# stelleg/caster-dta

Hardware: AMD Instinct MI355X
Metric: graph-pairs/sec (Davis-shaped protein+drug), encoders fwd+bwd (higher is better)
Workload: dtype f32; 1 GPU; davis_b64; pairs_per_gpu=64, residues_per_gpu=19200, protein_edges_per_gpu=57484, atoms_per_gpu=2560, drug_edges_per_gpu=7986, encoder=CASTER-DTA(2,2), pass=fwdbwd, activation_storage=fp32, scope=encoders, torch_compile=False, tunable_gemms=False, two_lane_head=False, train_mode=True, csr_build_in_step=True, hip_graph=True, kernels=mfma

## Files before the change

### caster-dta_amd/csrc/gine_quad_kernels.hip

```cpp
#include <hip/hip_runtime.h>
#include <stdlib.h>
#include <stdint.h>

#include "gvp_internal.h"
#include "gvp_quad.h"

using namespace gq;

namespace {

constexpr int WAVE = 64, TILE = 16;
constexpr int NTL = 4;

constexpr int pad4i(int x) { return (x + 3) / 4 * 4; }

__device__ __forceinline__ int opaque_lane(int lane) {
  asm volatile("" : "+v"(lane));
  return lane;
}

#ifndef CGVP_GINE_FENCE
#define CGVP_GINE_FENCE 1
#endif
#if CGVP_GINE_FENCE
// ... 15 lines not shown
__device__ unsigned long long* g_stamp_buf_gine = nullptr;
#define GSTAMP(slot)                                                                         \
  do {                                                                                       \
    __builtin_amdgcn_sched_barrier(0);                                                       \
    unsigned long long t_;                                                                   \
    asm volatile("s_waitcnt vmcnt(0) lgkmcnt(0)\n\ts_memtime %0\n\ts_waitcnt lgkmcnt(0)" : "=s"(t_)::"memory"); \
    __builtin_amdgcn_sched_barrier(0);                                                       \
    if (g_stamp_buf_gine && (threadIdx.x & 63) == 0)                                         \
      g_stamp_buf_gine[((size_t)blockIdx.x * (blockDim.x >> 6) + (threadIdx.x >> 6)) * 16 + (slot)] = t_;   \
  } while (0)
#else
#define GSTAMP(slot) do {} while (0)
#endif

template <int W, int VALID>
struct SegClip {
  static_assert(W % 16 == 0, "whole 16-channel tiles");
  static constexpr int steps = W / 4;
  static __host__ __device__ int col(int s, int g) {
    const int c = 16 * (s >> 2) + 4 * g + (s & 3);
    return c < VALID ? c : -1;
  }
};

struct GineQArgs {
  const float* x; const int64_t* ntypes; const float* eattr; const int64_t* etypes;
  const int32_t* rowptr; const int32_t* eperm; const int32_t* esrc; const int32_t* edst; int64_t N;
  const float* eps; const float* we; const float* be; const float* w0; const float* b0;
  const float* w1; const float* b1; float slope;
  const float* mask; gvp::RngArgs rng; const float* g_out; float* g_x; float* slab;
  const float* agg_in; const uint16_t* pos_in;
  float* g_edge; float* g_self;
  float* g_eattr; int eattr_accum;
};

template <int COUT>
__device__ __forceinline__ f4 gine_dropout(const float* mask, const gvp::RngArgs& rng, int64_t n, int mt, int g) {
  if (mask) return *reinterpret_cast<const f4*>(mask + n * COUT + 16 * mt + 4 * g);
  if (rng.seed) {
    float f[4];
    gvp::dropout4(rng.seed[0], rng.seed[1], rng.stream, n, 4 * mt + g, rng.p, f);
    return f4{f[0], f[1], f[2], f[3]};
  }
  return f4{1.f, 1.f, 1.f, 1.f};
}

template <int CIN, int CHID, int COUT, int NT, int NET, int ED, bool EG = false>
struct GineQ {
  static_assert(CHID % 16 == 0 && COUT % 16 == 0 && COUT <= 64, "hidden / output widths are whole 16-channel tiles (<= 4 output tiles)");
  static constexpr int KE = NET + ED, XW = CIN - NT, CINP = (CIN + 15) / 16 * 16;
  static constexpr int MI = CINP / 16, MH = CHID / 16, MO = COUT / 16;
  static constexpr int L_EPS = 0, L_W0 = 1, L_B0 = L_W0 + CHID * CIN, L_W1 = L_B0 + CHID, L_B1 = L_W1 + COUT * CHID,
                       L_WE = L_B1 + COUT, L_BE = L_WE + CIN * KE, L_SIZE = L_BE + CIN, BLK = pad4i(L_SIZE);
  typedef SegClip<CINP, CIN> KIn;
  typedef Seg<P1, 0, CHID> KHid;
  typedef Seg<P1, 0, COUT> KOut;
  typedef Seg<P2, 0, KE> KFeat;
  static_assert(KFeat::steps <= 4, "bond one-hot + features fit one slot tile");
  typedef Gemm<P1, CIN, KE, KFeat> GE;
  typedef Gemm<P1, CHID, CIN, KIn> G0;
  typedef Gemm<P1, COUT, CHID, KHid> G1;
  typedef GemmT<KHid, KOut, CHID> G1T;
  typedef GemmT<KIn, KHid, CIN> G0T;
  typedef GemmT<KFeat, KIn, KE> GET;
  static_assert(GET::MT == 1, "d eattr is one output tile");
  static constexpr int F_E = 0, F_0 = F_E + GE::NFRAG * 64, F_0T = F_0 + G0::NFRAG * 64, F_1 = F_0T + G0T::NFRAG * 64,
// ... 282 lines not shown
#pragma unroll
      for (int mt = 0; mt < MI; ++mt) {
        f4 ag;
        if (SAVED) {
          ag = *reinterpret_cast<const f4*>(a.agg_in + (valid ? n : n0) * CINP + 16 * mt + 4 * g);
          if (!valid) ag = zero;
        } else {
          ag = *reinterpret_cast<const f4*>(rows + i * CINP + 16 * mt + 4 * g);
        }
#pragma unroll
        for (int r = 0; r < 4; ++r) h[mt][r] = fmaf(eps1, xi[mt][r], ag[r]);
      }
      float bh[1][Q::KIn::steps];
#pragma unroll
      for (int s = 0; s < Q::KIn::steps; ++s) bh[0][s] = h[s >> 2][s & 3];
      f4 tpre[MH], t[MH];
#pragma unroll
      for (int mt = 0; mt < MH; ++mt) {
        f4 acc[1] = {*reinterpret_cast<const f4*>(frag + Q::V_B0 + 16 * mt + 4 * g)};
        apply<typename Q::G0, 1>(frag + Q::F_0, mt, bh, acc, lane);
        tpre[mt] = acc[0];
#pragma unroll
        for (int r = 0; r < 4; ++r) t[mt][r] = acc[0][r] > 0.f ? acc[0][r] : acc[0][r] * a.slope;
      }
      float bt[1][Q::KHid::steps];
#pragma unroll
      for (int s = 0; s < Q::KHid::steps; ++s) bt[0][s] = t[s >> 2][s & 3];
      f4 dy[MO];
#pragma unroll
      for (int mt = 0; mt < MO; ++mt) {
        f4 acc[1] = {*reinterpret_cast<const f4*>(frag + Q::V_B1 + 16 * mt + 4 * g)};
        apply<typename Q::G1, 1>(frag + Q::F_1, mt, bt, acc, lane);
        f4 gy = *reinterpret_cast<const f4*>(a.g_out + (valid ? n : n0) * COUT + 16 * mt + 4 * g);
        gy = gy * gine_dropout<COUT>(a.mask, a.rng, valid ? n : n0, mt, g);
        if (!valid) gy = zero;
#pragma unroll
        for (int r = 0; r < 4; ++r) dy[mt][r] = gy[r] * (acc[0][r] > 0.f ? 1.f : a.slope);
      }
      float bdy[1][Q::KOut::steps];
#pragma unroll
      for (int s = 0; s < Q::KOut::steps; ++s) bdy[0][s] = dy[s >> 2][s & 3];
      f4 dtp[MH];
#pragma unroll
      for (int mt = 0; mt < MH; ++mt) {
        f4 acc[1] = {zero};
        apply<typename Q::G1T, 1>(frag + Q::F_1T, mt, bdy, acc, lane);
#pragma unroll
        for (int r = 0; r < 4; ++r) dtp[mt][r] = acc[0][r] * (tpre[mt][r] > 0.f ? 1.f : a.slope);
      }
      float bdt[1][Q::KHid::steps];
#pragma unroll
      for (int s = 0; s < Q::KHid::steps; ++s) bdt[0][s] = dtp[s >> 2][s & 3];
      f4 dh[MI];
#pragma unroll
      for (int mt = 0; mt < MI; ++mt) {
        f4 acc[1] = {zero};
        apply<typename Q::G0T, 1>(frag + Q::F_0T, mt, bdt, acc, lane);
        dh[mt] = acc[0];
      }
      GSTAMP(3);
      {
        f4 AT[MO], BT[MH];
        transpose_slots<Q::KOut::steps>(bdy[0], AT, lane, tscr);
        transpose_slots<Q::KHid::steps>(bt[0], BT, lane, tscr);
        dw1_band<Q, 0>(AT, BT, blk, lane);
        dw1_band<Q, 1>(AT, BT, blk, lane);
// ... 141 lines not shown
#pragma unroll
          for (int r = 0; r < 4; ++r) {
            const int c = 16 * mt + 4 * g + r;
            tot[r] = row_total(dm[mt][r]);
            q[r] = blk + Q::L_BE + c;
            on[r] = i == 15 && c < CIN;
          }
          add_where<AccPriv, 4>(q, on, tot);
        }
      }
    }
    WAVE_LDS_SYNC();
  }
  GSTAMP(6);
  for (int off = 32; off > 0; off >>= 1) acc_eps += __shfl_down(acc_eps, off);
  if (lane0 == 0) blk[Q::L_EPS] += acc_eps;
  __syncthreads();
  float* out = a.slab + (size_t)blockIdx.x * Q::L_SIZE;
  for (int k = threadIdx.x; k < Q::L_SIZE; k += GQ_TPB) {
    float s = 0.f;
#pragma unroll
    for (int ww = 0; ww < GQ_WPB; ++ww) s += blocks[ww * Q::BLK + k];
    out[k] = s;
  }
  GSTAMP(7);
}

struct GineFArgs {
  const float* x; const int64_t* ntypes; const float* eattr; const int64_t* etypes;
  const int32_t* rowptr; const int32_t* eperm; const int32_t* esrc; const int32_t* edst; int64_t N;
  const float* eps; const float* we; const float* be; const float* w0; const float* b0;
  const float* w1; const float* b1; float slope; const float* mask; gvp::RngArgs rng; float* out;
  float* agg_out; uint16_t* pos_out;
};
#ifndef CGVP_GINE_FWD_WAVES
#define CGVP_GINE_FWD_WAVES 8
#endif
constexpr int GF_WPB = CGVP_GINE_FWD_WAVES, GF_TPB = WAVE * GF_WPB;

template <int CIN, int CHID, int COUT, int NT, int NET, int ED>
__global__ __launch_bounds__(GF_TPB) void gine_quad_fwd_kernel(GineFArgs a) {
  typedef GineQ<CIN, CHID, COUT, NT, NET, ED> Q;
  constexpr int KE = Q::KE, XW = Q::XW, CINP = Q::CINP, MI = Q::MI, MH = Q::MH, MO = Q::MO;
  constexpr int FE = 0, F0 = FE + Q::GE::NFRAG * 64, F1 = F0 + Q::G0::NFRAG * 64, VBE = F1 + Q::G1::NFRAG * 64,
                VB0 = VBE + CINP, VB1 = VB0 + CHID, FSZ = VB1 + COUT;
  extern __shared__ __attribute__((aligned(16))) float lds[];
  float* frag = lds;
  const int lane0 = threadIdx.x & 63, w = threadIdx.x >> 6;
  float* rows = frag + FSZ + w * Q::ROWS;
  stage_fragments<typename Q::GE, GF_TPB>(frag + FE, a.we);
  stage_fragments<typename Q::G0, GF_TPB>(frag + F0, a.w0);
  stage_fragments<typename Q::G1, GF_TPB>(frag + F1, a.w1);
  stage_biases<CIN, CINP, CHID, COUT, GF_TPB>(frag + VBE, frag + VB0, frag + VB1, a.be, a.b0, a.b1);
  __syncthreads();

  const f4 zero = {0.f, 0.f, 0.f, 0.f};
  const float eps1 = 1.0f + a.eps[0];
  const int64_t ntiles = (a.N + TILE - 1) / TILE;
  for (int64_t tile = (int64_t)blockIdx.x * GF_WPB + w; tile < ntiles; tile += (int64_t)gridDim.x * GF_WPB) {
    const int64_t n0 = tile * TILE;
    const int nn = (int)((a.N - n0 < TILE) ? (a.N - n0) : TILE);
    const int32_t e0 = a.rowptr[n0], e1 = a.rowptr[n0 + nn];
    for (int k = lane0; k < Q::ROWS / 4; k += WAVE) reinterpret_cast<f4*>(rows)[k] = zero;
    WAVE_LDS_SYNC();
    for (int32_t c0 = e0; c0 < e1; c0 += NTL * TILE) {
      const int lane = opaque_lane(lane0), i = lane & 15, g = lane >> 4;
// ... 44 lines not shown
    }
    {
      const int lane = opaque_lane(lane0), i = lane & 15, g = lane >> 4;
      const bool valid = i < nn;
      const int64_t n = n0 + i;
      float bh[1][Q::KIn::steps];
      f4 xi[MI];
      node_inputs<Q, CIN, NT, G_PIN>(a, n, valid, n0, g, xi);
#pragma unroll
      for (int mt = 0; mt < MI; ++mt) {
        const f4 ag = *reinterpret_cast<const f4*>(rows + i * CINP + 16 * mt + 4 * g);
        if (a.agg_out && valid) *reinterpret_cast<f4*>(a.agg_out + n * CINP + 16 * mt + 4 * g) = ag;
#pragma unroll
        for (int r = 0; r < 4; ++r) bh[0][4 * mt + r] = fmaf(eps1, xi[mt][r], ag[r]);
      }
      float bt[1][Q::KHid::steps];
#pragma unroll
      for (int mt = 0; mt < MH; ++mt) {
        f4 acc[1] = {*reinterpret_cast<const f4*>(frag + VB0 + 16 * mt + 4 * g)};
        apply<typename Q::G0, 1>(frag + F0, mt, bh, acc, lane);
#pragma unroll
        for (int r = 0; r < 4; ++r) bt[0][4 * mt + r] = acc[0][r] > 0.f ? acc[0][r] : acc[0][r] * a.slope;
      }
#pragma unroll
      for (int mt = 0; mt < MO; ++mt) {
        f4 acc[1] = {*reinterpret_cast<const f4*>(frag + VB1 + 16 * mt + 4 * g)};
        apply<typename Q::G1, 1>(frag + F1, mt, bt, acc, lane);
        f4 y;
#pragma unroll
        for (int r = 0; r < 4; ++r) y[r] = acc[0][r] > 0.f ? acc[0][r] : acc[0][r] * a.slope;
        if (valid) {
          y = y * gine_dropout<COUT>(a.mask, a.rng, n, mt, g);
          *reinterpret_cast<f4*>(a.out + n * COUT + 16 * mt + 4 * g) = y;
        }
      }
    }
    WAVE_LDS_SYNC();
  }
}

template <int CIN, int CHID, int COUT, int NT, int NET, int ED>
int launch_fwd(GineFArgs& a, hipStream_t st) {
  typedef GineQ<CIN, CHID, COUT, NT, NET, ED> Q;
  const int64_t tiles = (a.N + TILE - 1) / TILE;
  int64_t wgs = (tiles + GF_WPB - 1) / GF_WPB;
  static const int cap = [] {
    const char* e = getenv("CGVP_GINE_FWD_WGS");
    const int v = e ? atoi(e) : 0;
    return v >= 1 ? v : 1024;
  }();
  const int G = (int)(wgs < 1 ? 1 : (wgs > cap ? cap : wgs));
  const size_t lds = (size_t)((Q::GE::NFRAG + Q::G0::NFRAG + Q::G1::NFRAG) * 64 + Q::CINP + CHID + COUT + GF_WPB * Q::ROWS) * sizeof(float);
  CGVP_SET_DYN_LDS_ONCE((gine_quad_fwd_kernel<CIN, CHID, COUT, NT, NET, ED>), lds);
  hipLaunchKernelGGL((gine_quad_fwd_kernel<CIN, CHID, COUT, NT, NET, ED>), dim3(G), dim3(GF_TPB), lds, st, a);
  return 0;
}

template <int CIN, int CHID, int COUT, int NT, int NET, int ED>
int launch(GineQArgs& a, int cap, int* rows, int* row_len, hipStream_t st) {
  typedef GineQ<CIN, CHID, COUT, NT, NET, ED> Q;
  constexpr int GQ_WPB = Q::WPB, GQ_TPB = Q::TPB;
  const int64_t tiles = (a.N + TILE - 1) / TILE;
  int64_t wgs = (tiles + GQ_WPB - 1) / GQ_WPB;
  const int G = (int)(wgs < 1 ? 1 : (wgs > cap ? cap : wgs));
  if (a.g_eattr) {
    typedef GineQ<CIN, CHID, COUT, NT, NET, ED, true> QE;
    static_assert(QE::TPB == Q::TPB && QE::L_SIZE == Q::L_SIZE, "same workgroup shape and slab row");
    const size_t ldse = (size_t)QE::LDS_FLOATS * sizeof(float);
    if (a.g_edge) {
      if (!(a.agg_in && a.pos_in)) return CGVP_ERR_NONDETERMINISTIC;
      CGVP_SET_DYN_LDS_ONCE((gine_quad_bwd_kernel<CIN, CHID, COUT, NT, NET, ED, true, true, true>), ldse);
      hipLaunchKernelGGL((gine_quad_bwd_kernel<CIN, CHID, COUT, NT, NET, ED, true, true, true>), dim3(G), dim3(GQ_TPB), ldse, st, a);
    } else if (a.agg_in && a.pos_in) {
      CGVP_SET_DYN_LDS_ONCE((gine_quad_bwd_kernel<CIN, CHID, COUT, NT, NET, ED, true, false, true>), ldse);
      hipLaunchKernelGGL((gine_quad_bwd_kernel<CIN, CHID, COUT, NT, NET, ED, true, false, true>), dim3(G), dim3(GQ_TPB), ldse, st, a);
    } else {
      CGVP_SET_DYN_LDS_ONCE((gine_quad_bwd_kernel<CIN, CHID, COUT, NT, NET, ED, false, false, true>), ldse);
      hipLaunchKernelGGL((gine_quad_bwd_kernel<CIN, CHID, COUT, NT, NET, ED, false, false, true>), dim3(G), dim3(GQ_TPB), ldse, st, a);
    }
    *rows = G;
    *row_len = Q::L_SIZE;
    return 0;
  }
  const size_t lds = (size_t)Q::LDS_FLOATS * sizeof(float);
  if (a.g_edge) {
    if (!(a.agg_in && a.pos_in)) return CGVP_ERR_NONDETERMINISTIC;
    CGVP_SET_DYN_LDS_ONCE((gine_quad_bwd_kernel<CIN, CHID, COUT, NT, NET, ED, true, true>), lds);
    hipLaunchKernelGGL((gine_quad_bwd_kernel<CIN, CHID, COUT, NT, NET, ED, true, true>), dim3(G), dim3(GQ_TPB), lds, st, a);
  } else if (a.agg_in && a.pos_in) {
    CGVP_SET_DYN_LDS_ONCE((gine_quad_bwd_kernel<CIN, CHID, COUT, NT, NET, ED, true>), lds);
    hipLaunchKernelGGL((gine_quad_bwd_kernel<CIN, CHID, COUT, NT, NET, ED, true>), dim3(G), dim3(GQ_TPB), lds, st, a);
  } else {
    CGVP_SET_DYN_LDS_ONCE((gine_quad_bwd_kernel<CIN, CHID, COUT, NT, NET, ED, false>), lds);
    hipLaunchKernelGGL((gine_quad_bwd_kernel<CIN, CHID, COUT, NT, NET, ED, false>), dim3(G), dim3(GQ_TPB), lds, st, a);
  }
  *rows = G;
  *row_len = Q::L_SIZE;
  return 0;
}

}

namespace quad {

int gine_bwd(int cin, int chid, int cout, int nt, int net, int ed, const float* x, const int64_t* ntypes,
             const float* eattr, const int64_t* etypes, const int32_t* rowptr, const int32_t* eperm,
             const int32_t* esrc, const int32_t* edst, int64_t N, const cgvp_gine_w* w, float slope,
             const float* mask, gvp::RngArgs rng, const float* g_out, float* g_x, float* slab, int max_workgroups,
             int* rows, int* row_len, hipStream_t st, const float* agg_in, const uint16_t* pos_in,
             float* g_edge, float* g_self, float* g_eattr, int eattr_accum) {
  const int cap = max_workgroups <= 0 ? kGineBwdDefaultGrid : (max_workgroups > kGineBwdMaxGrid ? kGineBwdMaxGrid : max_workgroups);
  if (((uintptr_t)agg_in & 15) || ((uintptr_t)pos_in & 1)) return CGVP_ERR_BAD_ARG;
  GineQArgs a{x, ntypes, eattr, etypes, rowptr, eperm, esrc, edst, N, w->eps, w->we, w->be, w->w0, w->b0,
              w->w1, w->b1, slope, mask, rng, g_out, g_x, slab, agg_in, pos_in, g_edge, g_self, g_eattr, eattr_accum};
  if (cin == 52 && chid == 16 && cout == 16 && nt == 11 && net == 5 && ed == 9) return launch<52, 16, 16, 11, 5, 9>(a, cap, rows, row_len, st);
  if (cin == 52 && chid == 16 && cout == 16 && nt == 0 && net == 5 && ed == 9) return launch<52, 16, 16, 0, 5, 9>(a, cap, rows, row_len, st);
  if (cin == 16 && chid == 64 && cout == 64 && nt == 0 && net == 5 && ed == 9) return launch<16, 64, 64, 0, 5, 9>(a, cap, rows, row_len, st);
  if (cin == 16 && chid == 16 && cout == 16 && nt == 0 && net == 5 && ed == 9) return launch<16, 16, 16, 0, 5, 9>(a, cap, rows, row_len, st);
  return CGVP_ERR_UNSUPPORTED_DIMS;
}

int gine_fwd(int cin, int chid, int cout, int nt, int net, int ed, const float* x, const int64_t* ntypes,
             const float* eattr, const int64_t* etypes, const int32_t* rowptr, const int32_t* eperm,
             const int32_t* esrc, const int32_t* edst, int64_t N, const cgvp_gine_w* w, float slope,
             const float* mask, gvp::RngArgs rng, float* out, float* agg_out, uint16_t* pos_out, hipStream_t st) {
  if ((uintptr_t)agg_out & 15) return CGVP_ERR_BAD_ARG;
  GineFArgs a{x, ntypes, eattr, etypes, rowptr, eperm, esrc, edst, N, w->eps, w->we, w->be, w->w0, w->b0,
              w->w1, w->b1, slope, mask, rng, out, agg_out, pos_out};
  if (cin == 52 && chid == 16 && cout == 16 && nt == 11 && net == 5 && ed == 9) return launch_fwd<52, 16, 16, 11, 5, 9>(a, st);
  if (cin == 52 && chid == 16 && cout == 16 && nt == 0 && net == 5 && ed == 9) return launch_fwd<52, 16, 16, 0, 5, 9>(a, st);
  if (cin == 16 && chid == 64 && cout == 64 && nt == 0 && net == 5 && ed == 9) return launch_fwd<16, 64, 64, 0, 5, 9>(a, st);
  if (cin == 16 && chid == 16 && cout == 16 && nt == 0 && net == 5 && ed == 9) return launch_fwd<16, 16, 16, 0, 5, 9>(a, st);
  return 1;
}

}

#ifdef CGVP_STAMPS
extern "C" int cgvp_debug_set_stamp_buffer_gine(unsigned long long* buf) {
  return (int)hipMemcpyToSymbol(HIP_SYMBOL(g_stamp_buf_gine), &buf, sizeof(buf));
}
#endif
```

### caster-dta_amd/csrc/gvp_internal.h

```cpp
#pragma once
#include <hip/hip_runtime.h>
#include <stdint.h>

#include "../../include/caster_gvp.h"
#include "gvp_math.h"
#include "gvp_rng.h"

constexpr int POLICY_F32 = 0, POLICY_BF16 = 1, POLICY_GVPDEF = 2, POLICY_LINEAR = 3;

struct QuadOffsets {
  int emb, conv0, node0, layer_stride, head, total;
  int embT, convT0, nodeT0, layerT_stride, headT;
};

#ifndef CGVP_BWD_MAX_GRID
#define CGVP_BWD_MAX_GRID 240
#endif
constexpr int kBwdMaxGrid = CGVP_BWD_MAX_GRID;

#include <atomic>
#define CGVP_SET_DYN_LDS_ONCE(FN, BYTES)                                                                                      \
  do {                                                                                                                        \
    static std::atomic<uint64_t> cgvp_done_{0};                                                                               \
    int cgvp_dev_ = 0;                                                                                                        \
// ... 29 lines not shown
                    int bf16, hipStream_t st);
int head_bwd(const float* img_head, const float* imgT_head, const float* h_out, const float* g_out, int64_t N,
             float* g_h_out, float* slab, int* grid, int bf16, hipStream_t st);
int node_head_bwd(const float* img_head, const float* imgT_head, const float* h_out, const float* g_out, float* g_h_out,
                  float* head_slab, const float* img_node, const float* imgT_node, const float* h, const float* dh,
                  const float* mask0, const float* mask1, gvp::RngArgs rng, int64_t N, float* g_dh, float* g_h,
                  float* zero_rows, float* slab, int* grid, int bf16, hipStream_t st);
int conv_bwd(int nt_edge, const float* img, const float* imgT, const float* h, const float* e_emb,
             const int32_t* rowptr, const int32_t* esrc, const int32_t* edst, int64_t N, int64_t E, int mean,
             const float* g_dh, float* g_src, float* g_dst, float* g_e, float* slab, int* grid, int bf16, hipStream_t st,
             float* g_edge = nullptr, float* slot = nullptr);
int conv_bwd_max_waves();
int64_t src_index_work_ints(int64_t N, int64_t E);
int src_index(const int32_t* rowptr, const int32_t* esrc, int64_t N, int64_t E, int32_t* sptr, int32_t* spos,
              int32_t* work, hipStream_t st);
int src_sum(int width, const float* rows, const float* self, const int32_t* sptr, const int32_t* spos,
            const int32_t* rowptr, const float* slot, int64_t waves, int64_t N, float* out, hipStream_t st);
struct DetBufs { const int32_t* sptr; const int32_t* spos; float* rows; float* slot; };
int conv_bwd_entry(const cgvp_dims* dims, const cgvp_layout* layout, const float* image, int32_t layer,
                   const float* h, const float* e_emb, const int32_t* rowptr, const int32_t* esrc,
                   const int32_t* edst, int64_t N, int64_t E, int32_t aggr_mean, const float* g_dh, float* g_src,
                   int32_t g_src_zeroed, float* g_dst, float* g_e, float* grad_params, float* workspace,
                   cgvp_segment* segs, int32_t* nsegs, void* stream, const DetBufs* det);
bool deterministic_env();
int edge_embed_bwd(int nt_edge, const float* img, const float* imgT, const float* e_s, const float* e_v,
                   const int64_t* etypes, const int32_t* eperm, int64_t E, const float* const* g_e, int n_g,
                   float* g_e_s, float* g_e_v, float* slab, int* grid, int bf16, hipStream_t st);
constexpr int kEdgeRow = 36;
int node_embed_bwd(int nt_node, const float* img, const float* imgT, const float* x_s, const float* x_v,
                   const int64_t* ntypes, int64_t N, const float* g_up0, const float* g_up1, const float* g_up2,
                   float* g_x_s, float* g_x_v, float* slab, int* grid, int bf16, hipStream_t st);
constexpr int kGineBwdMaxGrid = 256;
constexpr int kGineBwdDefaultGrid = 16;
int gine_bwd(int cin, int chid, int cout, int nt, int net, int ed, const float* x, const int64_t* ntypes,
             const float* eattr, const int64_t* etypes, const int32_t* rowptr, const int32_t* eperm,
             const int32_t* esrc, const int32_t* edst, int64_t N, const cgvp_gine_w* w, float slope,
             const float* mask, gvp::RngArgs rng, const float* g_out, float* g_x, float* slab, int max_workgroups, int* rows,
             int* row_len, hipStream_t st, const float* agg_in = nullptr, const uint16_t* pos_in = nullptr,
             float* g_edge = nullptr, float* g_self = nullptr,
             float* g_eattr = nullptr, int eattr_accum = 0);
int gine_fwd(int cin, int chid, int cout, int nt, int net, int ed, const float* x, const int64_t* ntypes,
             const float* eattr, const int64_t* etypes, const int32_t* rowptr, const int32_t* eperm,
             const int32_t* esrc, const int32_t* edst, int64_t N, const cgvp_gine_w* w, float slope,
             const float* mask, gvp::RngArgs rng, float* out, float* agg_out, uint16_t* pos_out, hipStream_t st);
int reduce_slab(const float* slab, int rows, int stride, int col0, int len, float* dst, hipStream_t st);
int reduce_segments(const cgvp_segment* segs, int nsegs, float* grad_params, hipStream_t st, int overwrite = 0,
                    bool store_only = false);
int bwd_block_sizes(int nt_node, int nt_edge, int* emb, int* conv_edge, int* conv_total, int* node, int* head);
void zero_words(void* p, size_t words, hipStream_t s);
int csr_build(const int64_t* edge_index, int64_t N, int64_t E, int32_t* rowptr, int32_t* eperm, int32_t* esrc,
              int32_t* edst, int32_t* work, int work_is_zero, int32_t* ids_scratch, unsigned long long* rng_state,
              unsigned long long* rng_out, hipStream_t stream);
}
```

### caster-dta_amd/csrc/pass_api.hip

```cpp
#include <hip/hip_runtime.h>
#include <stdint.h>
#include <stdlib.h>

#include <atomic>
#include <mutex>
#include <vector>

#include "gvp_internal.h"

namespace {

struct TimedLaunch { hipEvent_t a, b; int kind; };
std::atomic<bool> g_timing{false};
std::mutex g_timed_mutex;
std::vector<TimedLaunch> g_timed;
struct Timed {
  hipStream_t st; bool on; TimedLaunch t;
  Timed(int kind, void* stream) : st((hipStream_t)stream), on(g_timing.load(std::memory_order_relaxed)) {
    if (!on) return;
    t.kind = kind;
    if (hipEventCreate(&t.a) != hipSuccess || hipEventCreate(&t.b) != hipSuccess) { on = false; return; }
    (void)hipEventRecord(t.a, st);
  }
  ~Timed() {
// ... 353 lines not shown
                                      g_dh, g_h, g_src, grad_params, region(), segs + nseg, &cnt, stream))
      return rc;
    nseg += cnt;
    {
      Timed timed(1, stream);
      if (int rc = quad::conv_bwd_entry(dims, layout, image, l, row(l), e_emb, rowptr, esrc, edst, N, E, aggr_mean, g_dh, g_src,
                                        1, g_dst, g_e + (int64_t)l * bw.g_e_stride, grad_params, region(), segs + nseg, &cnt,
                                        stream, det ? &db : nullptr))
        return rc;
    }
    nseg += cnt;
    up0 = g_h ? g_h : g_dh; up1 = g_src; up2 = g_dst;
  }
  if (int rc = cgvp_node_embed_bwd(dims, layout, image, batch->x_s, batch->x_v, batch->ntypes, N, up0, up1, up2, g_x_s, g_x_v,
                                   grad_params, region(), segs + nseg, &cnt, stream))
    return rc;
  nseg += cnt;
  if (E > 0) {
    const float* ge[16];
    if (nc > 16) return CGVP_ERR_UNSUPPORTED_DIMS;
    for (int l = 0; l < nc; ++l) ge[l] = g_e + (int64_t)l * bw.g_e_stride;
    if (int rc = cgvp_edge_embed_bwd(dims, layout, image, batch->e_s, batch->e_v, batch->etypes, eperm, E, ge, nc,
                                     g_e_s, g_e_v, grad_params, region(), segs + nseg, &cnt, stream))
      return rc;
    nseg += cnt;
  } else {
    quad::zero_words(grad_params + layout->edge_gvp, (size_t)(layout->conv0 - layout->edge_gvp), st);
  }
  if (det) quad::reduce_segments(segs, nseg, grad_params, st, 1, true);
  else if (int rc = cgvp_bwd_reduce(segs, nseg, grad_params, 1, stream)) return rc;
  return launch_status();
}

int cgvp_gine_fwd_workspace(const cgvp_gine_cfg* cfg, int64_t N, int64_t E, int32_t save_state, cgvp_gine_fwd_ws* out) {
  if (int rc = check_gine_cfg(cfg)) return rc;
  if (!out || N < 0 || E < 0) return CGVP_ERR_BAD_ARG;
  const int L = cfg->num_layers;
  Bump b;
  out->seed = b.take(16);
  for (int l = 0; l < CGVP_GINE_MAX_LAYERS; ++l) out->hidden[l] = out->agg[l] = out->pos[l] = 0;
  if (save_state) {
    for (int l = 0; l < L - 1; ++l) out->hidden[l] = b.take(N * cfg->widths[l + 1] * 4);
    for (int l = 0; l < L; ++l) {
      out->agg[l] = b.take(N * ((cfg->widths[l] + 15) / 16 * 16) * 4);
      out->pos[l] = b.take((E > 0 ? E : 1) * 8);
    }
  } else {
    int maxw = 1;
    for (int l = 1; l < L; ++l) maxw = cfg->widths[l] > maxw ? cfg->widths[l] : maxw;
    const int64_t a = b.take(N * maxw * 4), c = b.take(N * maxw * 4);
    for (int l = 0; l < L - 1; ++l) out->hidden[l] = (l & 1) ? c : a;
  }
  out->rowptr = b.take((N + 1) * 4);
  out->eperm = b.take((E > 0 ? E : 1) * 4);
  out->esrc = b.take((E > 0 ? E : 1) * 4);
  out->edst = b.take((E > 0 ? E : 1) * 4);
  out->saved = b.off;
  out->ids_scratch = b.take((E > 0 ? E : 1) * 4);
  out->total = b.off;
  return 0;
}

int cgvp_gine_forward_pass(const cgvp_gine_cfg* cfg, const cgvp_gine_w* w, const cgvp_gine_batch* batch, float dropout_p,
                           uint64_t* rng_state, const float* const* masks, int32_t* csr_counters, void* workspace,
                           int32_t save_state, int32_t variant, float* out, void* stream) {
  if (!cfg || !w || !batch || !workspace || ((uintptr_t)workspace & 255)) return CGVP_ERR_BAD_ARG;
  const int64_t N = batch->num_nodes, E = batch->num_edges;
  cgvp_gine_fwd_ws ws;
  if (int rc = cgvp_gine_fwd_workspace(cfg, N, E, save_state, &ws)) return rc;
  if (!(dropout_p >= 0.f && dropout_p < 1.f)) return CGVP_ERR_BAD_ARG;
  const int L = cfg->num_layers;
  const bool drop = dropout_p > 0.f && save_state && L > 1;
  const bool draw = drop && !masks;
  if (draw && !rng_state) return CGVP_ERR_BAD_ARG;
  const bool tables = has_tables(batch);
// ... 2 lines not shown
  hipStream_t st = (hipStream_t)stream;
  uint64_t* seed = at<uint64_t>(workspace, ws.seed);
  const int32_t* rowptr = tables ? batch->rowptr : at<int32_t>(workspace, ws.rowptr);
  const int32_t* eperm = tables ? batch->eperm : at<int32_t>(workspace, ws.eperm);
  const int32_t* esrc = tables ? batch->esrc : at<int32_t>(workspace, ws.esrc);
  const int32_t* edst = tables ? batch->edst : at<int32_t>(workspace, ws.edst);
  if (!tables) {
    if (int rc = quad::csr_build(batch->edge_index, N, E, at<int32_t>(workspace, ws.rowptr), at<int32_t>(workspace, ws.eperm),
                                 at<int32_t>(workspace, ws.esrc), at<int32_t>(workspace, ws.edst), csr_counters, 1,
                                 at<int32_t>(workspace, ws.ids_scratch),
                                 draw ? reinterpret_cast<unsigned long long*>(rng_state) : nullptr,
                                 draw ? reinterpret_cast<unsigned long long*>(seed) : nullptr, st))
      return rc;
  } else if (draw) {
    if (int rc = cgvp_rng_next(rng_state, seed, stream)) return rc;
  }
  if (N == 0) return 0;
  const float* x = batch->x;
  for (int l = 0; l < L; ++l) {
    const bool first = l == 0, lastl = l == L - 1;
    float* y = lastl ? out : at<float>(workspace, ws.hidden[l]);
    cgvp_rng rng{draw ? seed : nullptr, dropout_p, l};
    const bool dl = drop && !lastl;
    bool done = false;
    if (save_state) {
      if (((uintptr_t)x & 15) || ((uintptr_t)y & 15)) return CGVP_ERR_BAD_ARG;
      gvp::RngArgs ra{(dl && draw) ? reinterpret_cast<const unsigned long long*>(seed) : nullptr, dropout_p, l};
      if (!(dl && draw)) ra = gvp::RngArgs{nullptr, 0.f, 0};
      const int rc = quad::gine_fwd(cfg->widths[l], cfg->widths[l + 1], cfg->widths[l + 1], first ? cfg->num_ntypes : 0,
                                    cfg->num_etypes, cfg->edge_dim, x, first ? batch->ntypes : nullptr, batch->eattr,
                                    batch->etypes, rowptr, eperm, esrc, edst, N, w + l, cfg->act_slope,
                                    (dl && masks) ? masks[l] : nullptr, ra, y,
                                    gine_recompute() ? nullptr : at<float>(workspace, ws.agg[l]),
                                    gine_recompute() ? nullptr : at<uint16_t>(workspace, ws.pos[l]), st);
      if (rc < 0 || rc > 1) return rc;
      done = rc == 0;
    }
    if (!done)
      if (int rc = cgvp_gine_conv_fwd(x, first ? batch->ntypes : nullptr, first ? cfg->num_ntypes : 0, batch->eattr, batch->etypes,
                                      cfg->num_etypes, cfg->edge_dim, rowptr, eperm, esrc, edst, N, E, cfg->widths[l],
                                      cfg->widths[l + 1], cfg->widths[l + 1], w + l, cfg->act_slope,
                                      (dl && masks) ? masks[l] : nullptr, (dl && draw) ? &rng : nullptr, variant, y, stream))
        return rc;
    x = y;
  }
  return launch_status();
}

int64_t cgvp_gine_bwd_workspace_bytes(const cgvp_gine_cfg* cfg, int64_t N, int64_t E) {
  if (int rc = check_gine_cfg(cfg)) return rc;
  if (N < 0 || E < 0) return CGVP_ERR_BAD_ARG;
  GineBwdWs w;
  gine_bwd_layout(cfg, N, &w);
  return w.total;
}

int64_t cgvp_gine_bwd_workspace_bytes_ex(const cgvp_gine_cfg* cfg, int64_t N, int64_t E, int32_t flags) {
  if (int rc = check_gine_cfg(cfg)) return rc;
  if (N < 0 || E < 0) return CGVP_ERR_BAD_ARG;
  GineBwdWs w;
  gine_bwd_layout(cfg, N, &w, E, det_mode(flags));
  return w.total;
}

int cgvp_gine_backward_pass(const cgvp_gine_cfg* cfg, const cgvp_gine_w* w, const cgvp_gine_batch* batch, float dropout_p,
                            const float* const* masks, const void* fwd_workspace, const float* g_out, void* bwd_workspace,
                            float* grad_flat, float* g_x, int32_t max_workgroups, void* stream) {
// ... 12 lines not shown
int cgvp_gine_backward_pass_eattr(const cgvp_gine_cfg* cfg, const cgvp_gine_w* w, const cgvp_gine_batch* batch, float dropout_p,
                                  const float* const* masks, const void* fwd_workspace, const float* g_out, void* bwd_workspace,
                                  float* grad_flat, float* g_x, float* g_eattr, int32_t max_workgroups, int32_t flags,
                                  void* stream) {
  const bool det = det_mode(flags);
  if (det && gine_recompute()) return CGVP_ERR_NONDETERMINISTIC;
  if (!cfg || !w || !batch || !fwd_workspace || !bwd_workspace || !grad_flat) return CGVP_ERR_BAD_ARG;
  if (((uintptr_t)fwd_workspace & 255) || ((uintptr_t)bwd_workspace & 255)) return CGVP_ERR_BAD_ARG;
  const int64_t N = batch->num_nodes, E = batch->num_edges;
  cgvp_gine_fwd_ws ws;
  if (int rc = cgvp_gine_fwd_workspace(cfg, N, E, 1, &ws)) return rc;
  GineBwdWs bw;
  gine_bwd_layout(cfg, N, &bw, E, det);
  const int L = cfg->num_layers;
  const int ke = cfg->num_etypes + cfg->edge_dim;
  hipStream_t st = (hipStream_t)stream;
  int64_t total = 0;
  int loff[CGVP_GINE_MAX_LAYERS];
  for (int l = 0; l < L; ++l) { loff[l] = (int)total; total += gine_layer_floats(cfg->widths[l], cfg->widths[l + 1], cfg->widths[l + 1], ke); }
  if (N == 0) {
    quad::zero_words(grad_flat, (size_t)total, st);
    return launch_status();
  }
  if (!g_out) return CGVP_ERR_BAD_ARG;
  const bool drop = dropout_p > 0.f && L > 1;
  const bool draw = drop && !masks;
  const uint64_t* seed = at<uint64_t>(fwd_workspace, ws.seed);
  const bool tables = has_tables(batch);
  const int32_t* rowptr = tables ? batch->rowptr : at<int32_t>(fwd_workspace, ws.rowptr);
  const int32_t* eperm = tables ? batch->eperm : at<int32_t>(fwd_workspace, ws.eperm);
  const int32_t* esrc = tables ? batch->esrc : at<int32_t>(fwd_workspace, ws.esrc);
  const int32_t* edst = tables ? batch->edst : at<int32_t>(fwd_workspace, ws.edst);
  float* slabs = at<float>(bwd_workspace, bw.slabs);
  float* gx = at<float>(bwd_workspace, bw.gx);
  const DetWs& dw = bw.det_ws;
  if (det) {
    if (int rc = quad::src_index(rowptr, esrc, N, E, at<int32_t>(bwd_workspace, dw.sptr), at<int32_t>(bwd_workspace, dw.spos),
                                 at<int32_t>(bwd_workspace, dw.work), st))
      return rc;
  } else {
    if (L > 1) quad::zero_words(gx, (size_t)(L - 1) * bw.gx_floats, st);
    if (g_x) quad::zero_words(g_x, (size_t)N * (cfg->widths[0] - cfg->num_ntypes), st);
  }
  cgvp_segment segs[CGVP_GINE_MAX_LAYERS];
  const float* g = g_out;
  for (int l = L - 1; l >= 0; --l) {
    const bool first = l == 0;
    const float* x = first ? batch->x : at<float>(fwd_workspace, ws.hidden[l - 1]);
    float* gxl = first ? g_x : gx + (int64_t)(l - 1) * bw.gx_floats;
    const bool dl = drop && l < L - 1;
    gvp::RngArgs ra{(dl && draw) ? reinterpret_cast<const unsigned long long*>(seed) : nullptr, dropout_p, l};
    if (!(dl && draw)) ra = gvp::RngArgs{nullptr, 0.f, 0};
    const float* mask = (dl && masks) ? masks[l] : nullptr;
    if (((uintptr_t)g & 15) || ((uintptr_t)mask & 15)) return CGVP_ERR_BAD_ARG;
    int rows = 0, row_len = 0;
    float* slab = slabs + (int64_t)l * bw.slab_floats;
    if (int rc = quad::gine_bwd(cfg->widths[l], cfg->widths[l + 1], cfg->widths[l + 1], first ? cfg->num_ntypes : 0,
                                cfg->num_etypes, cfg->edge_dim, x, first ? batch->ntypes : nullptr, batch->eattr, batch->etypes,
                                rowptr, eperm, esrc, edst, N, w + l, cfg->act_slope, mask, ra, g, gxl, slab, max_workgroups,
                                &rows, &row_len, st, gine_recompute() ? nullptr : at<float>(fwd_workspace, ws.agg[l]),
                                gine_recompute() ? nullptr : at<uint16_t>(fwd_workspace, ws.pos[l]),
                                det ? at<float>(bwd_workspace, dw.rows) : nullptr,
                                (det && gxl) ? at<float>(bwd_workspace, dw.extra) : nullptr,
                                g_eattr, l < L - 1))
      return rc;
    if (det && gxl)
      if (int rc = quad::src_sum(cfg->widths[l] - (first ? cfg->num_ntypes : 0), at<float>(bwd_workspace, dw.rows),
                                 at<float>(bwd_workspace, dw.extra), at<int32_t>(bwd_workspace, dw.sptr),
                                 at<int32_t>(bwd_workspace, dw.spos), rowptr, nullptr, 0, N, gxl, st))
        return rc;
    segs[l] = cgvp_segment{slab, rows, row_len, 0,
                           gine_layer_floats(cfg->widths[l], cfg->widths[l + 1], cfg->widths[l + 1], ke), loff[l]};
    g = gxl;
  }
  if (det) quad::reduce_segments(segs, L, grad_flat, st, 1, true);
  else quad::reduce_segments(segs, L, grad_flat, st, 1);
  return launch_status();
}

int cgvp_debug_kernel_timing(int32_t enable) {
  g_timing.store(enable != 0, std::memory_order_relaxed);
  return 0;
}

int cgvp_debug_kernel_times(float* ms, int32_t* kinds, int32_t capacity) {
  int n = 0;
  std::vector<TimedLaunch> taken;
  {
    std::lock_guard<std::mutex> lock(g_timed_mutex);
    taken.swap(g_timed);
  }
  for (const TimedLaunch& t : taken) {
    float v = 0.f;
    (void)hipEventSynchronize(t.b);
    (void)hipEventElapsedTime(&v, t.a, t.b);
    if (n < capacity && ms && kinds) { ms[n] = v; kinds[n] = t.kind; }
    ++n;
// ... 8 lines not shown
```

### caster-dta_amd/gvp_hip/autograd_ops.py

```python
from __future__ import annotations

import ctypes as C
import math
import os
from typing import List, Tuple

import torch
from torch import Tensor

from . import _lib, ops
from .ops import _act, _f32, _i64, _ptr, _stream

MROW = 20
_CFG_FIELDS = ("node_in_s", "node_in_v", "edge_in_s", "edge_in_v", "hidden_s", "hidden_v", "edge_hidden_s",
               "edge_hidden_v", "out_s")
CFG_NTN, CFG_NTE, CFG_NC, CFG_MEAN, CFG_LEN = 9, 10, 11, 12, 13


PINNED_MASKS = None


def draw_seed(device):
    return torch.randint(0, 1 << 62, (2,), dtype=torch.int64, device=device)

# ... 45 lines not shown
        img = int(_lib.lib().cgvp_lba_image_floats(C.byref(dims), C.byref(layout)))
        if img < 0:
            _lib.check(img, "cgvp_lba_image_floats")
        hit = _DIMS[key] = (dims, layout, img)
    return hit


def flat_arena(params):
    p0 = params[0]
    st, off = p0.untyped_storage(), p0.storage_offset()
    o = off
    for p in params:
        if p.untyped_storage().data_ptr() != st.data_ptr() or p.storage_offset() != o or not p.is_contiguous():
            return torch.cat([q.detach().reshape(-1) for q in params])
        o += p.numel()
    return torch.empty(0, dtype=p0.dtype, device=p0.device).set_(st, off, (o - off,), (1,))


def _up(v, a=256):
    return (v + a - 1) // a * a


def lba_fwd_ws_bytes(N, E, num_convs, image_floats, esize, save_state):
    rows = 2 * num_convs + 1 if save_state else 3
    e1 = E if E > 0 else 1
    return (_up(16) + _up(image_floats * 4) + _up(rows * (N + N % 2) * ops.ROW * esize) + _up((E + 1) * ops.EROW * esize)
            + _up((N + 1) * 4) + 3 * _up(e1 * 4))


def gine_fwd_ws_bytes(N, E, widths, save_state, saved_only=False):
    L = len(widths) - 1
    e1 = E if E > 0 else 1
    if save_state:
        hidden = sum(_up(N * widths[l + 1] * 4) for l in range(L - 1))
        hidden += sum(_up(N * ((widths[l] + 15) // 16 * 16) * 4) + _up(e1 * 8) for l in range(L))
    else:
        hidden = 2 * _up(N * max([1] + list(widths[1:L])) * 4)
    return _up(16) + hidden + _up((N + 1) * 4) + (3 if saved_only else 4) * _up(e1 * 4)


def _csr_ptrs(csr):
    if len(csr) == 0:
        return 0, 0, 0, 0
    if len(csr) != 4 or any(t.dtype != torch.int32 or not t.is_cuda for t in csr):
        raise ValueError("csr must be [] or the four int32 CUDA tables rowptr, eperm, esrc, edst")
    return tuple(t.data_ptr() for t in csr)


def _batch(cls, nodes, edges, edge_index, csr, N, E):
    ptr = lambda t: 0 if t is None else t.data_ptr()
    return cls(N, E, *map(ptr, nodes), *(ptr(t) if E > 0 else 0 for t in edges),
               ptr(edge_index) if (E > 0 and not csr) else 0, *_csr_ptrs(csr))


def _dropout(p, save_state, shapes, dev):
    if p <= 0 or not save_state or not shapes:
        return None, False
    if PINNED_MASKS is None:
        return None, True
    return [PINNED_MASKS(count, n, width, p, dev) for count, n, width in shapes], False


def _record_draw(kind, ws, draw):
    if draw:
        _LAST_WS[kind] = (ws, 0)


# ... 485 lines not shown
```

Baseline: 280,600 graph-pairs/sec.

## Fuse hidden-gradient zeroing into GINE forward/backward kernels and tune bwd grid

Removes the separate zero_words launch that cleared the hidden-layer gradient buffers before the non-deterministic backward. The forward kernel now zeroes a per-layer gradient buffer, newly allocated in the forward workspace next to each saved hidden activation, as it writes the output. The backward kernel re-zeroes that buffer after reading g_out so it is clean for the next step. It also picks a larger default backward grid when the tile count is small. The cost is extra forward workspace memory and extra stores in both kernels, and correctness now depends on the buffer starting out zeroed and on forward always running before backward.

```diff
diff --git a/caster-dta_amd/csrc/gine_quad_kernels.hip b/caster-dta_amd/csrc/gine_quad_kernels.hip
--- a/caster-dta_amd/csrc/gine_quad_kernels.hip
+++ b/caster-dta_amd/csrc/gine_quad_kernels.hip
@@ -71,6 +71,7 @@
   const float* agg_in; const uint16_t* pos_in;
   float* g_edge; float* g_self;
   float* g_eattr; int eattr_accum;
+  float* g_rezero;
 };
 
 template <int COUT>
@@ -419,6 +420,7 @@
         f4 acc[1] = {*reinterpret_cast<const f4*>(frag + Q::V_B1 + 16 * mt + 4 * g)};
         apply<typename Q::G1, 1>(frag + Q::F_1, mt, bt, acc, lane);
         f4 gy = *reinterpret_cast<const f4*>(a.g_out + (valid ? n : n0) * COUT + 16 * mt + 4 * g);
+        if (a.g_rezero && valid) *reinterpret_cast<f4*>(a.g_rezero + n * COUT + 16 * mt + 4 * g) = zero;
         gy = gy * gine_dropout<COUT>(a.mask, a.rng, valid ? n : n0, mt, g);
         if (!valid) gy = zero;
 #pragma unroll
@@ -626,6 +628,7 @@
   const float* eps; const float* we; const float* be; const float* w0; const float* b0;
   const float* w1; const float* b1; float slope; const float* mask; gvp::RngArgs rng; float* out;
   float* agg_out; uint16_t* pos_out;
+  float* zero_out;
 };
 #ifndef CGVP_GINE_FWD_WAVES
 #define CGVP_GINE_FWD_WAVES 8
@@ -736,6 +739,7 @@
         if (valid) {
           y = y * gine_dropout<COUT>(a.mask, a.rng, n, mt, g);
           *reinterpret_cast<f4*>(a.out + n * COUT + 16 * mt + 4 * g) = y;
+          if (a.zero_out) *reinterpret_cast<f4*>(a.zero_out + n * COUT + 16 * mt + 4 * g) = zero;
         }
       }
     }
@@ -766,6 +770,7 @@
   constexpr int GQ_WPB = Q::WPB, GQ_TPB = Q::TPB;
   const int64_t tiles = (a.N + TILE - 1) / TILE;
   int64_t wgs = (tiles + GQ_WPB - 1) / GQ_WPB;
+  if (cap <= 0) cap = wgs <= quad::kGineBwdOneTileGrid ? quad::kGineBwdOneTileGrid : quad::kGineBwdDefaultGrid;
   const int G = (int)(wgs < 1 ? 1 : (wgs > cap ? cap : wgs));
   if (a.g_eattr) {
     typedef GineQ<CIN, CHID, COUT, NT, NET, ED, true> QE;
@@ -812,11 +817,11 @@
              const int32_t* esrc, const int32_t* edst, int64_t N, const cgvp_gine_w* w, float slope,
              const float* mask, gvp::RngArgs rng, const float* g_out, float* g_x, float* slab, int max_workgroups,
              int* rows, int* row_len, hipStream_t st, const float* agg_in, const uint16_t* pos_in,
-             float* g_edge, float* g_self, float* g_eattr, int eattr_accum) {
-  const int cap = max_workgroups <= 0 ? kGineBwdDefaultGrid : (max_workgroups > kGineBwdMaxGrid ? kGineBwdMaxGrid : max_workgroups);
+             float* g_edge, float* g_self, float* g_eattr, int eattr_accum, float* g_rezero) {
+  const int cap = max_workgroups <= 0 ? 0 : (max_workgroups > kGineBwdMaxGrid ? kGineBwdMaxGrid : max_workgroups);
   if (((uintptr_t)agg_in & 15) || ((uintptr_t)pos_in & 1)) return CGVP_ERR_BAD_ARG;
   GineQArgs a{x, ntypes, eattr, etypes, rowptr, eperm, esrc, edst, N, w->eps, w->we, w->be, w->w0, w->b0,
-              w->w1, w->b1, slope, mask, rng, g_out, g_x, slab, agg_in, pos_in, g_edge, g_self, g_eattr, eattr_accum};
+              w->w1, w->b1, slope, mask, rng, g_out, g_x, slab, agg_in, pos_in, g_edge, g_self, g_eattr, eattr_accum, g_rezero};
   if (cin == 52 && chid == 16 && cout == 16 && nt == 11 && net == 5 && ed == 9) return launch<52, 16, 16, 11, 5, 9>(a, cap, rows, row_len, st);
   if (cin == 52 && chid == 16 && cout == 16 && nt == 0 && net == 5 && ed == 9) return launch<52, 16, 16, 0, 5, 9>(a, cap, rows, row_len, st);
   if (cin == 16 && chid == 64 && cout == 64 && nt == 0 && net == 5 && ed == 9) return launch<16, 64, 64, 0, 5, 9>(a, cap, rows, row_len, st);
@@ -827,10 +832,11 @@
 int gine_fwd(int cin, int chid, int cout, int nt, int net, int ed, const float* x, const int64_t* ntypes,
              const float* eattr, const int64_t* etypes, const int32_t* rowptr, const int32_t* eperm,
              const int32_t* esrc, const int32_t* edst, int64_t N, const cgvp_gine_w* w, float slope,
-             const float* mask, gvp::RngArgs rng, float* out, float* agg_out, uint16_t* pos_out, hipStream_t st) {
-  if ((uintptr_t)agg_out & 15) return CGVP_ERR_BAD_ARG;
+             const float* mask, gvp::RngArgs rng, float* out, float* agg_out, uint16_t* pos_out, hipStream_t st,
+             float* zero_out) {
+  if (((uintptr_t)agg_out & 15) || ((uintptr_t)zero_out & 15)) return CGVP_ERR_BAD_ARG;
   GineFArgs a{x, ntypes, eattr, etypes, rowptr, eperm, esrc, edst, N, w->eps, w->we, w->be, w->w0, w->b0,
-              w->w1, w->b1, slope, mask, rng, out, agg_out, pos_out};
+              w->w1, w->b1, slope, mask, rng, out, agg_out, pos_out, zero_out};
   if (cin == 52 && chid == 16 && cout == 16 && nt == 11 && net == 5 && ed == 9) return launch_fwd<52, 16, 16, 11, 5, 9>(a, st);
   if (cin == 52 && chid == 16 && cout == 16 && nt == 0 && net == 5 && ed == 9) return launch_fwd<52, 16, 16, 0, 5, 9>(a, st);
   if (cin == 16 && chid == 64 && cout == 64 && nt == 0 && net == 5 && ed == 9) return launch_fwd<16, 64, 64, 0, 5, 9>(a, st);
diff --git a/caster-dta_amd/csrc/gvp_internal.h b/caster-dta_amd/csrc/gvp_internal.h
--- a/caster-dta_amd/csrc/gvp_internal.h
+++ b/caster-dta_amd/csrc/gvp_internal.h
@@ -85,17 +85,20 @@
                    float* g_x_s, float* g_x_v, float* slab, int* grid, int bf16, hipStream_t st);
 constexpr int kGineBwdMaxGrid = 256;
 constexpr int kGineBwdDefaultGrid = 16;
+constexpr int kGineBwdOneTileGrid = 24;
 int gine_bwd(int cin, int chid, int cout, int nt, int net, int ed, const float* x, const int64_t* ntypes,
              const float* eattr, const int64_t* etypes, const int32_t* rowptr, const int32_t* eperm,
              const int32_t* esrc, const int32_t* edst, int64_t N, const cgvp_gine_w* w, float slope,
              const float* mask, gvp::RngArgs rng, const float* g_out, float* g_x, float* slab, int max_workgroups, int* rows,
              int* row_len, hipStream_t st, const float* agg_in = nullptr, const uint16_t* pos_in = nullptr,
              float* g_edge = nullptr, float* g_self = nullptr,
-             float* g_eattr = nullptr, int eattr_accum = 0);
+             float* g_eattr = nullptr, int eattr_accum = 0,
+             float* g_rezero = nullptr);
 int gine_fwd(int cin, int chid, int cout, int nt, int net, int ed, const float* x, const int64_t* ntypes,
              const float* eattr, const int64_t* etypes, const int32_t* rowptr, const int32_t* eperm,
              const int32_t* esrc, const int32_t* edst, int64_t N, const cgvp_gine_w* w, float slope,
-             const float* mask, gvp::RngArgs rng, float* out, float* agg_out, uint16_t* pos_out, hipStream_t st);
+             const float* mask, gvp::RngArgs rng, float* out, float* agg_out, uint16_t* pos_out, hipStream_t st,
+             float* zero_out = nullptr);
 int reduce_slab(const float* slab, int rows, int stride, int col0, int len, float* dst, hipStream_t st);
 int reduce_segments(const cgvp_segment* segs, int nsegs, float* grad_params, hipStream_t st, int overwrite = 0,
                     bool store_only = false);
diff --git a/caster-dta_amd/csrc/pass_api.hip b/caster-dta_amd/csrc/pass_api.hip
--- a/caster-dta_amd/csrc/pass_api.hip
+++ b/caster-dta_amd/csrc/pass_api.hip
@@ -409,6 +409,10 @@
   return launch_status();
 }
 
+static int64_t gine_ghidden(const cgvp_gine_cfg* cfg, const cgvp_gine_fwd_ws& ws, int64_t N, int l) {
+  return ws.hidden[l] + up(N * cfg->widths[l + 1] * 4, 256);
+}
+
 int cgvp_gine_fwd_workspace(const cgvp_gine_cfg* cfg, int64_t N, int64_t E, int32_t save_state, cgvp_gine_fwd_ws* out) {
   if (int rc = check_gine_cfg(cfg)) return rc;
   if (!out || N < 0 || E < 0) return CGVP_ERR_BAD_ARG;
@@ -417,7 +421,10 @@
   out->seed = b.take(16);
   for (int l = 0; l < CGVP_GINE_MAX_LAYERS; ++l) out->hidden[l] = out->agg[l] = out->pos[l] = 0;
   if (save_state) {
-    for (int l = 0; l < L - 1; ++l) out->hidden[l] = b.take(N * cfg->widths[l + 1] * 4);
+    for (int l = 0; l < L - 1; ++l) {
+      out->hidden[l] = b.take(N * cfg->widths[l + 1] * 4);
+      b.take(N * cfg->widths[l + 1] * 4);
+    }
     for (int l = 0; l < L; ++l) {
       out->agg[l] = b.take(N * ((cfg->widths[l] + 15) / 16 * 16) * 4);
       out->pos[l] = b.take((E > 0 ? E : 1) * 8);
@@ -486,7 +493,8 @@
                                     batch->etypes, rowptr, eperm, esrc, edst, N, w + l, cfg->act_slope,
                                     (dl && masks) ? masks[l] : nullptr, ra, y,
                                     gine_recompute() ? nullptr : at<float>(workspace, ws.agg[l]),
-                                    gine_recompute() ? nullptr : at<uint16_t>(workspace, ws.pos[l]), st);
+                                    gine_recompute() ? nullptr : at<uint16_t>(workspace, ws.pos[l]), st,
+                                    lastl ? nullptr : at<float>(workspace, gine_ghidden(cfg, ws, N, l)));
       if (rc < 0 || rc > 1) return rc;
       done = rc == 0;
     }
@@ -565,14 +573,16 @@
   const int32_t* esrc = tables ? batch->esrc : at<int32_t>(fwd_workspace, ws.esrc);
   const int32_t* edst = tables ? batch->edst : at<int32_t>(fwd_workspace, ws.edst);
   float* slabs = at<float>(bwd_workspace, bw.slabs);
-  float* gx = at<float>(bwd_workspace, bw.gx);
+  auto ghidden = [&](int l) {
+    return det ? at<float>(bwd_workspace, bw.gx) + (int64_t)l * bw.gx_floats
+               : const_cast<float*>(at<float>(fwd_workspace, gine_ghidden(cfg, ws, N, l)));
+  };
   const DetWs& dw = bw.det_ws;
   if (det) {
     if (int rc = quad::src_index(rowptr, esrc, N, E, at<int32_t>(bwd_workspace, dw.sptr), at<int32_t>(bwd_workspace, dw.spos),
                                  at<int32_t>(bwd_workspace, dw.work), st))
       return rc;
   } else {
-    if (L > 1) quad::zero_words(gx, (size_t)(L - 1) * bw.gx_floats, st);
     if (g_x) quad::zero_words(g_x, (size_t)N * (cfg->widths[0] - cfg->num_ntypes), st);
   }
   cgvp_segment segs[CGVP_GINE_MAX_LAYERS];
@@ -580,7 +590,7 @@
   for (int l = L - 1; l >= 0; --l) {
     const bool first = l == 0;
     const float* x = first ? batch->x : at<float>(fwd_workspace, ws.hidden[l - 1]);
-    float* gxl = first ? g_x : gx + (int64_t)(l - 1) * bw.gx_floats;
+    float* gxl = first ? g_x : ghidden(l - 1);
     const bool dl = drop && l < L - 1;
     gvp::RngArgs ra{(dl && draw) ? reinterpret_cast<const unsigned long long*>(seed) : nullptr, dropout_p, l};
     if (!(dl && draw)) ra = gvp::RngArgs{nullptr, 0.f, 0};
@@ -595,7 +605,8 @@
                                 gine_recompute() ? nullptr : at<uint16_t>(fwd_workspace, ws.pos[l]),
                                 det ? at<float>(bwd_workspace, dw.rows) : nullptr,
                                 (det && gxl) ? at<float>(bwd_workspace, dw.extra) : nullptr,
-                                g_eattr, l < L - 1))
+                                g_eattr, l < L - 1,
+                                (!det && l < L - 1) ? ghidden(l) : nullptr))
       return rc;
     if (det && gxl)
       if (int rc = quad::src_sum(cfg->widths[l] - (first ? cfg->num_ntypes : 0), at<float>(bwd_workspace, dw.rows),
diff --git a/caster-dta_amd/gvp_hip/autograd_ops.py b/caster-dta_amd/gvp_hip/autograd_ops.py
--- a/caster-dta_amd/gvp_hip/autograd_ops.py
+++ b/caster-dta_amd/gvp_hip/autograd_ops.py
@@ -101,7 +101,7 @@
     L = len(widths) - 1
     e1 = E if E > 0 else 1
     if save_state:
-        hidden = sum(_up(N * widths[l + 1] * 4) for l in range(L - 1))
+        hidden = sum(2 * _up(N * widths[l + 1] * 4) for l in range(L - 1))
         hidden += sum(_up(N * ((widths[l] + 15) // 16 * 16) * 4) + _up(e1 * 8) for l in range(L))
     else:
         hidden = 2 * _up(N * max([1] + list(widths[1:L])) * 4)
```

Result: no change. 282,200 graph-pairs/sec, median of 6 (+0.6%).
